# tdavchev/DESIRE

Hardware: AMD Instinct MI355X
Metric: agent-trajectory-samples/sec (K=20, T_pred=40) (higher is better)
Workload: dtype f32; 1 GPU; BASELINE configs[1]: SDD-like synthetic windows, 32 agent slots/window, K=20, T_obs=8/T_pred=40, H=128, L=128, fp32, posterior CVAE, IOC 1 refinement, social grid 4x4, scene grid 64x64x32; 512 windows/step/GPU; windows_per_gpu=512, rows_per_gpu=327680, parallelism=scene-sharded x1

## Files before the change

desire_amd/csrc/kernels_gemm.hip:

```cpp
#include "common.h"
#include "kernels.h"

#define KC 256
#define LDA_C (KC + 4)

template <int EPI, int NTW, int MT = 2>
__global__ __launch_bounds__(DS_WG, 2) void k_gemm_rows(GemmArgs a) {
    constexpr int TMR = 32 * MT;
    extern __shared__ __attribute__((aligned(16))) float smem[];
    const int lane = lane_id(), w = wave_id(), tid = threadIdx.x;
    const int row0 = blockIdx.x * TMR;
    DYN_N(a, M, row0)
    f32x16 acc[NTW][MT];
#pragma unroll
    for (int j = 0; j < NTW; ++j)
#pragma unroll
        for (int m = 0; m < MT; ++m) acc[j][m] = zero16();
    const float* a_lane = smem + (lane & 31) * LDA_C + 4 * (lane >> 5);

    for (int k0 = 0; k0 < a.K; k0 += KC) {
        const int kc = min(KC, a.K - k0);
        const int q = kc >> 2;
        for (int i = tid; i < TMR * q; i += DS_WG) {
            const int r = i / q, c4 = i - r * q;
            const int row = row0 + r;
            float4 v = make_float4(0.f, 0.f, 0.f, 0.f);
            if (row < a.M) v = *reinterpret_cast<const float4*>(a.A + (size_t)row * a.lda + k0 + c4 * 4);
            *reinterpret_cast<float4*>(smem + r * LDA_C + c4 * 4) = v;
        }
        __syncthreads();
#pragma unroll
        for (int j = 0; j < NTW; ++j) {
            const int nt = (blockIdx.y * NTW + j) * 4 + w;
            if (nt < a.NT)
                mma_groups<MT>(acc[j], a_lane, LDA_C, a.Bp + ((size_t)nt * a.G + (k0 >> 3)) * 64 + lane, kc >> 3);
        }
        __syncthreads();
    }
#pragma unroll
    for (int j = 0; j < NTW; ++j) {
        const int nt = (blockIdx.y * NTW + j) * 4 + w;
        if (nt >= a.NT) continue;
        const int col = nt * 32 + (lane & 31);
        if (col >= a.N) continue;
        float p0 = 0.f, p1 = 0.f;
        if (EPI == EPI_SCALE_SHIFT_ELU) { const int ch = col % a.chmod; p0 = a.p0[ch]; p1 = a.p1[ch]; }
        else if (EPI == EPI_ELUGRAD || EPI == EPI_SIGGRAD) p0 = a.p0[col % a.chmod];
        else if (EPI != EPI_NONE) p0 = a.p0[col];
#pragma unroll
        for (int m = 0; m < MT; ++m)
#pragma unroll
            for (int i = 0; i < 16; ++i) {
                const int row = row0 + m * 32 + acc_row(i);
                if (row >= a.M) continue;
                float v = acc[j][m][i];
                if (EPI == EPI_BIAS) v = v + p0;
                else if (EPI == EPI_BIAS_RELU) v = fmaxf(v + p0, 0.f);
                else if (EPI == EPI_SCALE_SHIFT_ELU) v = eluf_(v * p0 + p1);
                else if (EPI == EPI_ELUGRAD) { const float y = a.aux[(size_t)row * a.ldo + col]; v = v * (y > 0.f ? 1.0f : y + 1.0f) * p0; }
                else if (EPI == EPI_SIGGRAD) { const float y = a.aux[(size_t)row * a.ldo + col]; v = v * y * (1.0f - y) * p0; }
                a.out[(size_t)row * a.ldo + col] = v;
            }
    }
}

template <int NTW, int MT>
static void launch_gemm_rows_n(const GemmArgs& a, int epi, hipStream_t s) {
    constexpr int TMR = 32 * MT;
    dim3 grid((a.M + TMR - 1) / TMR, (a.NT + 4 * NTW - 1) / (4 * NTW));
    const size_t lds = TMR * LDA_C * sizeof(float);
    if (epi == EPI_NONE) launch_big_lds<k_gemm_rows<EPI_NONE, NTW, MT>>(grid, dim3(DS_WG), lds, s, a);
    else if (epi == EPI_ELUGRAD) launch_big_lds<k_gemm_rows<EPI_ELUGRAD, NTW, MT>>(grid, dim3(DS_WG), lds, s, a);
    else if (epi == EPI_SIGGRAD) launch_big_lds<k_gemm_rows<EPI_SIGGRAD, NTW, MT>>(grid, dim3(DS_WG), lds, s, a);
    else if (epi == EPI_BIAS) launch_big_lds<k_gemm_rows<EPI_BIAS, NTW, MT>>(grid, dim3(DS_WG), lds, s, a);
    else if (epi == EPI_BIAS_RELU) launch_big_lds<k_gemm_rows<EPI_BIAS_RELU, NTW, MT>>(grid, dim3(DS_WG), lds, s, a);
    else launch_big_lds<k_gemm_rows<EPI_SCALE_SHIFT_ELU, NTW, MT>>(grid, dim3(DS_WG), lds, s, a);
}
void launch_gemm_rows(const GemmArgs& a, int epi, hipStream_t s) {
    const int Msel = (a.dyn.cnt && a.M_hint > 0) ? a.M_hint : a.M;
    const long wgs = (long)((Msel + DS_TM - 1) / DS_TM) * ((a.NT + 15) / 16);
    if (wgs < 128) launch_gemm_rows_n<1, 1>(a, epi, s); else launch_gemm_rows_n<4, 2>(a, epi, s);
}

__global__ void k_reparam(const float* __restrict__ params, const float* __restrict__ eps,
                          float* __restrict__ z, int R, int L, int K, int mno, int posterior) {
    const int i = blockIdx.x * blockDim.x + threadIdx.x;
    if (i >= R * L) return;
    const int r = i / L, l = i - r * L;
    float e = eps[i];
    if (posterior) {
        const int a = agent_of_row(r, K, mno);
        const float mu = params[(size_t)a * 2 * L + l], ls = params[(size_t)a * 2 * L + L + l];
        e = mu + sqrtf(expf(ls)) * e;
    }
    z[i] = e;
}

void launch_reparam(const float* params, const float* eps, float* z, int R, int L, int K, int mno,
                    int posterior, hipStream_t s) {
    const int n = R * L;
    hipLaunchKernelGGL(k_reparam, dim3((n + 255) / 256), dim3(256), 0, s, params, eps, z, R, L, K, mno, posterior);
}

__global__ __launch_bounds__(DS_WG) void k_mask(MaskArgs a) {
    extern __shared__ __attribute__((aligned(16))) float smem[];
    const int lane = lane_id(), w = wave_id(), tid = threadIdx.x;
    const int row0 = blockIdx.x * DS_TM;
    DYN_P(a, row0)
    const int NT = a.H >> 5;
    f32x16 acc[2][2] = {{zero16(), zero16()}, {zero16(), zero16()}};
    const float* a_lane = smem + (lane & 31) * LDA_C + 4 * (lane >> 5);
    const int G = a.V >> 3;
    for (int k0 = 0; k0 < a.V; k0 += KC) {
        const int q = KC >> 2;
        for (int i = tid; i < DS_TM * q; i += DS_WG) {
            const int r = i / q, c4 = i - r * q;
            const int row = row0 + r;
            float4 v = make_float4(0.f, 0.f, 0.f, 0.f);
            if (row < a.R) v = *reinterpret_cast<const float4*>(a.xhat + (size_t)row * a.V + k0 + c4 * 4);
            *reinterpret_cast<float4*>(smem + r * LDA_C + c4 * 4) = v;
        }
        __syncthreads();
#pragma unroll
        for (int j = 0; j < 2; ++j) {
            const int nt = w + 4 * j;
            if (nt < NT) mma_groups<2>(acc[j], a_lane, LDA_C, a.Wp + ((size_t)nt * G + (k0 >> 3)) * 64 + lane, KC >> 3);
        }
        __syncthreads();
    }
    const int LDT = a.H + 4;
#pragma unroll
    for (int j = 0; j < 2; ++j) {
        const int nt = w + 4 * j;
        if (nt >= NT) continue;
        const int col = nt * 32 + (lane & 31);
        const float b = a.bias[col];
#pragma unroll
        for (int m = 0; m < 2; ++m)
#pragma unroll
            for (int i = 0; i < 16; ++i) {
                const float pv = fmaxf(acc[j][m][i] + b, 0.f);
                smem[(m * 32 + acc_row(i)) * LDT + col] = pv;
                if (a.sv_p && row0 + m * 32 + acc_row(i) < a.R) a.sv_p[(size_t)(row0 + m * 32 + acc_row(i)) * a.H + col] = pv;
            }
    }
    __syncthreads();
    const int r = tid >> 2, q4 = tid & 3;
    const int row = row0 + r;
    const int nv = a.H >> 4;
    float4* trow = reinterpret_cast<float4*>(smem + r * LDT);
    float mx = -3.0e38f;
    for (int j = 0; j < nv; ++j) { const float4 v = trow[4 * j + q4]; mx = fmaxf(mx, fmaxf(fmaxf(v.x, v.y), fmaxf(v.z, v.w))); }
    mx = fmaxf(mx, __shfl_xor(mx, 1));
    mx = fmaxf(mx, __shfl_xor(mx, 2));
    float sum = 0.f;
    for (int j = 0; j < nv; ++j) {
        float4 v = trow[4 * j + q4];
        v.x = expf(v.x - mx); v.y = expf(v.y - mx); v.z = expf(v.z - mx); v.w = expf(v.w - mx);
        trow[4 * j + q4] = v;
        const int c0 = 16 * j + 4 * q4;
        sum += (c0 < a.Hl ? v.x : 0.f) + (c0 + 1 < a.Hl ? v.y : 0.f) + (c0 + 2 < a.Hl ? v.z : 0.f) + (c0 + 3 < a.Hl ? v.w : 0.f);
    }
    sum += __shfl_xor(sum, 1);
    sum += __shfl_xor(sum, 2);
    if (row < a.R) {
        const int ag = agent_of_row(row, a.K, a.mno);
        const float inv = 1.0f / sum;
        const float4* hx = reinterpret_cast<const float4*>(a.Hx + (size_t)ag * a.ldhx);
        float4* xz = reinterpret_cast<float4*>(a.xz + (size_t)row * a.H);
        for (int j = 0; j < nv; ++j) {
            const float4 e = trow[4 * j + q4], hv = hx[4 * j + q4];
            xz[4 * j + q4] = make_float4(e.x * inv * hv.x, e.y * inv * hv.y, e.z * inv * hv.z, e.w * inv * hv.w);
        }
    }
}

void launch_mask(const MaskArgs& a, hipStream_t s) {
    const size_t lds = DS_TM * LDA_C * sizeof(float);
    launch_big_lds<k_mask>(dim3((a.R + DS_TM - 1) / DS_TM), dim3(DS_WG), lds, s, a);
}
```

Before: 2.624 million samples/s.

## Add single-chunk GEMM path with prefetched B heads and K-sized LDS stride

For GEMMs with K no larger than the chunk size, a new kernel variant stages the A rows once and then loops over N tiles one at a time. Each iteration prefetches the next tile's B fragment head (mma_begin/mma_run) while the current tile's epilogue runs, and only one accumulator set is live, which allows a higher occupancy bound. The LDS stride now tracks the actual K to shrink shared memory, and the epilogue takes a fast path with no bounds checks when the whole row tile is in range. Risks include reliance on the unseen mma_begin/mma_run helpers, inline asm scheduling barriers, and serialised N-tile iterations that lose some instruction-level parallelism.

```diff
diff --git a/desire_amd/csrc/kernels_gemm.hip b/desire_amd/csrc/kernels_gemm.hip
--- a/desire_amd/csrc/kernels_gemm.hip
+++ b/desire_amd/csrc/kernels_gemm.hip
@@ -2,79 +2,140 @@
 #include "kernels.h"
 
 #define KC 256
-#define LDA_C (KC + 4)
-
-template <int EPI, int NTW, int MT = 2>
-__global__ __launch_bounds__(DS_WG, 2) void k_gemm_rows(GemmArgs a) {
+static inline int lda_of(int K) { return (K < KC ? K : KC) + 4; }
+
+__device__ __forceinline__ void stage_rows(float* smem, int lds_ld, const float* __restrict__ A, int lda, int M, int row0, int rows, int k0, int kc) {
+    const int q = kc >> 2;
+    for (int i = threadIdx.x; i < rows * q; i += DS_WG) {
+        const int r = i / q, c4 = i - r * q;
+        const int row = row0 + r;
+        float4 v = make_float4(0.f, 0.f, 0.f, 0.f);
+        if (row < M) v = *reinterpret_cast<const float4*>(A + (size_t)row * lda + k0 + c4 * 4);
+        *reinterpret_cast<float4*>(smem + r * lds_ld + c4 * 4) = v;
+    }
+}
+
+struct EpiParams { float p0, p1; };
+template <int EPI>
+__device__ __forceinline__ EpiParams gemm_rows_params(const GemmArgs& a, int nt) {
+    const int col = nt * 32 + (lane_id() & 31);
+    EpiParams e{0.f, 0.f};
+    if (col >= a.N) return e;
+    if (EPI == EPI_SCALE_SHIFT_ELU) { const int ch = col % a.chmod; e.p0 = a.p0[ch]; e.p1 = a.p1[ch]; }
+    else if (EPI == EPI_ELUGRAD || EPI == EPI_SIGGRAD) e.p0 = a.p0[col % a.chmod];
+    else if (EPI != EPI_NONE) e.p0 = a.p0[col];
+    return e;
+}
+template <int EPI, int MT>
+__device__ __forceinline__ void gemm_rows_epilogue(const GemmArgs& a, const f32x16 (&acc)[MT], int nt, int row0, const EpiParams& e) {
+    const int lane = lane_id();
+    const int col = nt * 32 + (lane & 31);
+    if (col >= a.N) return;
+    const float p0 = e.p0, p1 = e.p1;
+    const int hi4 = 4 * (lane >> 5);
+    const unsigned voff = (unsigned)hi4 * (unsigned)a.ldo + (unsigned)col;
+    auto put = [&](int m, int i) {
+        const int rowu = row0 + m * 32 + (i & 3) + 8 * (i >> 2);
+        float v = acc[m][i];
+        if (EPI == EPI_BIAS) v = v + p0;
+        else if (EPI == EPI_BIAS_RELU) v = fmaxf(v + p0, 0.f);
+        else if (EPI == EPI_SCALE_SHIFT_ELU) v = eluf_(v * p0 + p1);
+        else if (EPI == EPI_ELUGRAD) { const float y = (a.aux + (size_t)rowu * a.ldo)[voff]; v = v * (y > 0.f ? 1.0f : y + 1.0f) * p0; }
+        else if (EPI == EPI_SIGGRAD) { const float y = (a.aux + (size_t)rowu * a.ldo)[voff]; v = v * y * (1.0f - y) * p0; }
+        (a.out + (size_t)rowu * a.ldo)[voff] = v;
+    };
+    if (row0 + 32 * MT <= a.M) {
+#pragma unroll
+        for (int m = 0; m < MT; ++m)
+#pragma unroll
+            for (int i = 0; i < 16; ++i) put(m, i);
+    } else {
+#pragma unroll
+        for (int m = 0; m < MT; ++m)
+#pragma unroll
+            for (int i = 0; i < 16; ++i)
+                if (row0 + m * 32 + (i & 3) + 8 * (i >> 2) + hi4 < a.M) put(m, i);
+    }
+}
+
+template <int EPI, int NTW, int MT, bool ONE>
+__global__ __launch_bounds__(DS_WG, ONE ? 4 : 2) void k_gemm_rows(GemmArgs a, int lds_ld) {
     constexpr int TMR = 32 * MT;
     extern __shared__ __attribute__((aligned(16))) float smem[];
-    const int lane = lane_id(), w = wave_id(), tid = threadIdx.x;
+    const int lane = lane_id(), w = wave_id();
     const int row0 = blockIdx.x * TMR;
     DYN_N(a, M, row0)
-    f32x16 acc[NTW][MT];
-#pragma unroll
-    for (int j = 0; j < NTW; ++j)
-#pragma unroll
-        for (int m = 0; m < MT; ++m) acc[j][m] = zero16();
-    const float* a_lane = smem + (lane & 31) * LDA_C + 4 * (lane >> 5);
-
-    for (int k0 = 0; k0 < a.K; k0 += KC) {
-        const int kc = min(KC, a.K - k0);
-        const int q = kc >> 2;
-        for (int i = tid; i < TMR * q; i += DS_WG) {
-            const int r = i / q, c4 = i - r * q;
-            const int row = row0 + r;
-            float4 v = make_float4(0.f, 0.f, 0.f, 0.f);
-            if (row < a.M) v = *reinterpret_cast<const float4*>(a.A + (size_t)row * a.lda + k0 + c4 * 4);
-            *reinterpret_cast<float4*>(smem + r * LDA_C + c4 * 4) = v;
-        }
+    const float* a_lane = smem + (lane & 31) * lds_ld + 4 * (lane >> 5);
+    if constexpr (ONE) {
+        const float* ap[MT];
+#pragma unroll
+        for (int m = 0; m < MT; ++m) ap[m] = a_lane + m * 32 * lds_ld;
+        const int G = a.K >> 3, nt0 = blockIdx.y * NTW * 4 + w;
+        MmaHead hd;
+        if (nt0 < a.NT) mma_begin(hd, a.Bp + (size_t)nt0 * a.G * 64 + lane, G);
+        __builtin_amdgcn_sched_barrier(0);
+        stage_rows(smem, lds_ld, a.A, a.lda, a.M, row0, TMR, 0, a.K);
         __syncthreads();
+#pragma unroll 1
+        for (int j = 0; j < NTW; ++j) {
+            const int nt = nt0 + 4 * j;
+            if (nt >= a.NT) break;
+            f32x16 acc[MT];
+#pragma unroll
+            for (int m = 0; m < MT; ++m) acc[m] = zero16();
+            const EpiParams e = gemm_rows_params<EPI>(a, nt);
+            mma_run<MT>(acc, ap, a.Bp + (size_t)nt * a.G * 64 + lane, G, hd);
+            asm volatile("" :: "v"(e.p0), "v"(e.p1));
+            if (j + 1 < NTW && nt + 4 < a.NT) mma_begin(hd, a.Bp + (size_t)(nt + 4) * a.G * 64 + lane, G);
+            __builtin_amdgcn_sched_barrier(0);
+            int r0 = row0;
+            asm volatile("" : "+s"(r0));
+            gemm_rows_epilogue<EPI, MT>(a, acc, nt, r0, e);
+        }
+    } else {
+        f32x16 acc[NTW][MT];
+#pragma unroll
+        for (int j = 0; j < NTW; ++j)
+#pragma unroll
+            for (int m = 0; m < MT; ++m) acc[j][m] = zero16();
+        for (int k0 = 0; k0 < a.K; k0 += KC) {
+            const int kc = min(KC, a.K - k0);
+            stage_rows(smem, lds_ld, a.A, a.lda, a.M, row0, TMR, k0, kc);
+            __syncthreads();
+#pragma unroll
+            for (int j = 0; j < NTW; ++j) {
+                const int nt = (blockIdx.y * NTW + j) * 4 + w;
+                if (nt < a.NT)
+                    mma_groups<MT>(acc[j], a_lane, lds_ld, a.Bp + ((size_t)nt * a.G + (k0 >> 3)) * 64 + lane, kc >> 3);
+            }
+            __syncthreads();
+        }
 #pragma unroll
         for (int j = 0; j < NTW; ++j) {
             const int nt = (blockIdx.y * NTW + j) * 4 + w;
-            if (nt < a.NT)
-                mma_groups<MT>(acc[j], a_lane, LDA_C, a.Bp + ((size_t)nt * a.G + (k0 >> 3)) * 64 + lane, kc >> 3);
-        }
-        __syncthreads();
-    }
-#pragma unroll
-    for (int j = 0; j < NTW; ++j) {
-        const int nt = (blockIdx.y * NTW + j) * 4 + w;
-        if (nt >= a.NT) continue;
-        const int col = nt * 32 + (lane & 31);
-        if (col >= a.N) continue;
-        float p0 = 0.f, p1 = 0.f;
-        if (EPI == EPI_SCALE_SHIFT_ELU) { const int ch = col % a.chmod; p0 = a.p0[ch]; p1 = a.p1[ch]; }
-        else if (EPI == EPI_ELUGRAD || EPI == EPI_SIGGRAD) p0 = a.p0[col % a.chmod];
-        else if (EPI != EPI_NONE) p0 = a.p0[col];
-#pragma unroll
-        for (int m = 0; m < MT; ++m)
-#pragma unroll
-            for (int i = 0; i < 16; ++i) {
-                const int row = row0 + m * 32 + acc_row(i);
-                if (row >= a.M) continue;
-                float v = acc[j][m][i];
-                if (EPI == EPI_BIAS) v = v + p0;
-                else if (EPI == EPI_BIAS_RELU) v = fmaxf(v + p0, 0.f);
-                else if (EPI == EPI_SCALE_SHIFT_ELU) v = eluf_(v * p0 + p1);
-                else if (EPI == EPI_ELUGRAD) { const float y = a.aux[(size_t)row * a.ldo + col]; v = v * (y > 0.f ? 1.0f : y + 1.0f) * p0; }
-                else if (EPI == EPI_SIGGRAD) { const float y = a.aux[(size_t)row * a.ldo + col]; v = v * y * (1.0f - y) * p0; }
-                a.out[(size_t)row * a.ldo + col] = v;
-            }
-    }
-}
-
+            int r0 = row0;
+            asm volatile("" : "+s"(r0));
+            if (nt < a.NT) gemm_rows_epilogue<EPI, MT>(a, acc[j], nt, r0, gemm_rows_params<EPI>(a, nt));
+        }
+    }
+}
+
+template <int NTW, int MT, bool ONE>
+static void launch_gemm_rows_f(const GemmArgs& a, int epi, hipStream_t s) {
+    constexpr int TMR = 32 * MT;
+    dim3 grid((a.M + TMR - 1) / TMR, (a.NT + 4 * NTW - 1) / (4 * NTW));
+    const int lds_ld = lda_of(a.K);
+    const size_t lds = (size_t)TMR * lds_ld * sizeof(float);
+    if (epi == EPI_NONE) launch_big_lds<k_gemm_rows<EPI_NONE, NTW, MT, ONE>>(grid, dim3(DS_WG), lds, s, a, lds_ld);
+    else if (epi == EPI_ELUGRAD) launch_big_lds<k_gemm_rows<EPI_ELUGRAD, NTW, MT, ONE>>(grid, dim3(DS_WG), lds, s, a, lds_ld);
+    else if (epi == EPI_SIGGRAD) launch_big_lds<k_gemm_rows<EPI_SIGGRAD, NTW, MT, ONE>>(grid, dim3(DS_WG), lds, s, a, lds_ld);
+    else if (epi == EPI_BIAS) launch_big_lds<k_gemm_rows<EPI_BIAS, NTW, MT, ONE>>(grid, dim3(DS_WG), lds, s, a, lds_ld);
+    else if (epi == EPI_BIAS_RELU) launch_big_lds<k_gemm_rows<EPI_BIAS_RELU, NTW, MT, ONE>>(grid, dim3(DS_WG), lds, s, a, lds_ld);
+    else launch_big_lds<k_gemm_rows<EPI_SCALE_SHIFT_ELU, NTW, MT, ONE>>(grid, dim3(DS_WG), lds, s, a, lds_ld);
+}
 template <int NTW, int MT>
 static void launch_gemm_rows_n(const GemmArgs& a, int epi, hipStream_t s) {
-    constexpr int TMR = 32 * MT;
-    dim3 grid((a.M + TMR - 1) / TMR, (a.NT + 4 * NTW - 1) / (4 * NTW));
-    const size_t lds = TMR * LDA_C * sizeof(float);
-    if (epi == EPI_NONE) launch_big_lds<k_gemm_rows<EPI_NONE, NTW, MT>>(grid, dim3(DS_WG), lds, s, a);
-    else if (epi == EPI_ELUGRAD) launch_big_lds<k_gemm_rows<EPI_ELUGRAD, NTW, MT>>(grid, dim3(DS_WG), lds, s, a);
-    else if (epi == EPI_SIGGRAD) launch_big_lds<k_gemm_rows<EPI_SIGGRAD, NTW, MT>>(grid, dim3(DS_WG), lds, s, a);
-    else if (epi == EPI_BIAS) launch_big_lds<k_gemm_rows<EPI_BIAS, NTW, MT>>(grid, dim3(DS_WG), lds, s, a);
-    else if (epi == EPI_BIAS_RELU) launch_big_lds<k_gemm_rows<EPI_BIAS_RELU, NTW, MT>>(grid, dim3(DS_WG), lds, s, a);
-    else launch_big_lds<k_gemm_rows<EPI_SCALE_SHIFT_ELU, NTW, MT>>(grid, dim3(DS_WG), lds, s, a);
+    if (a.K <= KC) launch_gemm_rows_f<NTW, MT, true>(a, epi, s); else launch_gemm_rows_f<NTW, MT, false>(a, epi, s);
 }
 void launch_gemm_rows(const GemmArgs& a, int epi, hipStream_t s) {
     const int Msel = (a.dyn.cnt && a.M_hint > 0) ? a.M_hint : a.M;
@@ -102,6 +163,8 @@
     hipLaunchKernelGGL(k_reparam, dim3((n + 255) / 256), dim3(256), 0, s, params, eps, z, R, L, K, mno, posterior);
 }
 
+#define MKC 256
+#define LDA_M (MKC + 4)
 __global__ __launch_bounds__(DS_WG) void k_mask(MaskArgs a) {
     extern __shared__ __attribute__((aligned(16))) float smem[];
     const int lane = lane_id(), w = wave_id(), tid = threadIdx.x;
@@ -109,22 +172,15 @@
     DYN_P(a, row0)
     const int NT = a.H >> 5;
     f32x16 acc[2][2] = {{zero16(), zero16()}, {zero16(), zero16()}};
-    const float* a_lane = smem + (lane & 31) * LDA_C + 4 * (lane >> 5);
+    const float* a_lane = smem + (lane & 31) * LDA_M + 4 * (lane >> 5);
     const int G = a.V >> 3;
-    for (int k0 = 0; k0 < a.V; k0 += KC) {
-        const int q = KC >> 2;
-        for (int i = tid; i < DS_TM * q; i += DS_WG) {
-            const int r = i / q, c4 = i - r * q;
-            const int row = row0 + r;
-            float4 v = make_float4(0.f, 0.f, 0.f, 0.f);
-            if (row < a.R) v = *reinterpret_cast<const float4*>(a.xhat + (size_t)row * a.V + k0 + c4 * 4);
-            *reinterpret_cast<float4*>(smem + r * LDA_C + c4 * 4) = v;
-        }
+    for (int k0 = 0; k0 < a.V; k0 += MKC) {
+        stage_rows(smem, LDA_M, a.xhat, a.V, a.R, row0, DS_TM, k0, MKC);
         __syncthreads();
 #pragma unroll
         for (int j = 0; j < 2; ++j) {
             const int nt = w + 4 * j;
-            if (nt < NT) mma_groups<2>(acc[j], a_lane, LDA_C, a.Wp + ((size_t)nt * G + (k0 >> 3)) * 64 + lane, KC >> 3);
+            if (nt < NT) mma_groups<2>(acc[j], a_lane, LDA_M, a.Wp + ((size_t)nt * G + (k0 >> 3)) * 64 + lane, MKC >> 3);
         }
         __syncthreads();
     }
@@ -176,6 +232,6 @@
 }
 
 void launch_mask(const MaskArgs& a, hipStream_t s) {
-    const size_t lds = DS_TM * LDA_C * sizeof(float);
+    const size_t lds = (size_t)DS_TM * (LDA_M > a.H + 4 ? LDA_M : a.H + 4) * sizeof(float);
     launch_big_lds<k_mask>(dim3((a.R + DS_TM - 1) / DS_TM), dim3(DS_WG), lds, s, a);
 }
```

Result: no change. 2.639 million samples/s, median of 6 (+0.6%).
